# dvillacis/BPLDenoising

Hardware: AMD Instinct MI355X
Metric: PDHG iters/sec (batched 128x128 images) (higher is better)
Workload: dtype f64; 1 GPU; 10x128x128 f64 batch, scalar alpha, 5000 PDHG iterations per step (denoise); images_per_gpu=10, tile_iters=8, tiles_per_launch=490, hipgraph=True, parallelism=images of one batch sharded, dp1

## Files before the change

bpldenoising_amd/csrc/pdhg_kernels.hpp:

```cpp
#pragma once
#include <hip/hip_runtime.h>

#include "tiling.hpp"

namespace bpltv {

constexpr size_t pdhg_lds_bytes(int RI, int RJ, size_t word = sizeof(double)) {
    return word * ((size_t)RJ * (RI + 1) + (size_t)(RJ + 1) * RI + (size_t)RJ * RI + RI + 1);
}

constexpr int TAB_STRIDE = 8;

struct PdhgArgs {
    const double* xin;
    const double* y1in;
    const double* y2in;
    double* xout;
    double* y1out;
    double* y2out;
    const double* f;
    const double* alpha;
    const double* tab;
    double rho;
    int am, an;
    int it0, nit;
    int M, N, O;
    int nTi, nTj, halo;
    int first;
    int img0;
    int Odata;
    int astride;
    int istride;
    int ntiles;
    int grid3d;
    int seg;
    int xcd;
    unsigned* phase = nullptr;
#ifdef BPLTV_EXPERIMENTS
    int dbg;
#endif
};

#ifdef BPLTV_EXPERIMENTS
#define BPLTV_DBG(A) ((A).dbg)
__device__ long long pdhg_tlog[2][4096];
#define PDHG_TLOG(A)                                                                                                   \
    if (((A).dbg & 1024) && threadIdx.x == 0 && blockIdx.x == 0 && blockIdx.y == 0 && blockIdx.z == 0)                  \
        pdhg_tlog[(A).img0 != 0][min(4095, ((A).it0 + (A).halo - 1) / max((A).halo, 1))] = (long long)wall_clock64();
#else
#define BPLTV_DBG(A) 0
#define PDHG_TLOG(A)
#endif

#define PDHG_PHASE_STAMP(A)                                                                              \
    if ((A).phase != nullptr && threadIdx.x == 0 && blockIdx.x == 0 && blockIdx.y == 0 && blockIdx.z == 0) \
        *(A).phase = (unsigned)(A).it0 + 1u;
#define PDHG_DECODE_BLOCK(A, imgl, ta, tb)                                   \
    PDHG_PHASE_STAMP(A)                                                      \
    PDHG_TLOG(A)                                                             \
    int imgl, ta, tb;                                                        \
    if ((A).grid3d) {                                                        \
        ta = (int)blockIdx.x; tb = (int)blockIdx.y; imgl = (int)blockIdx.z;  \
    } else {                                                                 \
        const int tilesPerImg_ = (A).nTi * (A).nTj;                          \
        int lin_ = (int)blockIdx.x;                                          \
        if ((A).xcd) {                                                       \
            const int q_ = (int)gridDim.x >> 3, r_ = (int)gridDim.x & 7;     \
            const int x_ = lin_ & 7, i_ = lin_ >> 3;                         \
            lin_ = x_ * q_ + (x_ < r_ ? x_ : r_) + i_;                       \
        }                                                                    \
        imgl = lin_ / tilesPerImg_;                                          \
        const int t_ = lin_ - imgl * tilesPerImg_;                           \
        ta = t_ % (A).nTi; tb = t_ / (A).nTi;                                \
    }
__device__ __forceinline__ size_t pdhg_data_image(const PdhgArgs& A, int img, int& fimg) {
    if (A.O == A.Odata) { fimg = img; return (size_t)img * A.istride; }
    fimg = img % A.Odata;
    return (size_t)(img / A.Odata) * A.astride;
}

__device__ __forceinline__ double alpha_at(const double* __restrict__ alpha, int am, int an, int M,
                                           int N, int i, int j) {
    if (am == 1 && an == 1) return alpha[0];
    if (am == M && an == N) return alpha[i + (size_t)M * j];
    return alpha[(int)(((long)i * am) / M) + (size_t)am * (int)(((long)j * an) / N)];
}

__device__ __forceinline__ double rsqrt_nr(double n2) {
    const unsigned long long u = 0x5FE6EB50C7B537A9ull - ((unsigned long long)__double_as_longlong(n2) >> 1);
    double r = __longlong_as_double((long long)u);
    const double h = 0.5 * n2;
#pragma unroll
    for (int k = 0; k < 4; ++k) {
        const double t = r * r;
        const double w = __builtin_fma(-h, t, 1.5);
        r = r * w;
    }
    return r;
}

__device__ __forceinline__ float rsqrt_nr(float n2) {
    const unsigned u = 0x5F375A86u - (__float_as_uint(n2) >> 1);
    float r = __uint_as_float(u);
    const float h = 0.5f * n2;
#pragma unroll
    for (int k = 0; k < 3; ++k) {
        const float t = r * r;
        const float w = __builtin_fmaf(-h, t, 1.5f);
        r = r * w;
    }
    return r;
}
__device__ __forceinline__ void rsqrt_nr_seed(double n2, double& r, double& h) {
    const unsigned long long u = 0x5FE6EB50C7B537A9ull - ((unsigned long long)__double_as_longlong(n2) >> 1);
    r = __longlong_as_double((long long)u);
    h = 0.5 * n2;
}
__device__ __forceinline__ void rsqrt_nr_seed(float n2, float& r, float& h) {
    r = __uint_as_float(0x5F375A86u - (__float_as_uint(n2) >> 1));
    h = 0.5f * n2;
}
__host__ __device__ constexpr int rsqrt_nr_steps(double) { return 4; }
__host__ __device__ constexpr int rsqrt_nr_steps(float) { return 3; }
__device__ __forceinline__ double pd_fma(double a, double b, double c) { return __builtin_fma(a, b, c); }
__device__ __forceinline__ float pd_fma(float a, float b, float c) { return __builtin_fmaf(a, b, c); }

template <typename T, int PI, int PJ, int TI, int TJ>
__global__ __launch_bounds__(TI* TJ) void pdhg_tile_kernel(PdhgArgs A) {
    constexpr int RI = PI * TI, RJ = PJ * TJ;
    constexpr int S1 = RI + 1;
    extern __shared__ __attribute__((aligned(16))) unsigned char pdhg_smem[];
    T* smem = reinterpret_cast<T*>(pdhg_smem);
    T* sy1 = smem;
    T* sy2 = smem + RJ * S1;
    T* sxb = smem + RJ * S1 + (RJ + 1) * RI;
    const T* __restrict__ Axin = reinterpret_cast<const T*>(A.xin);
    const T* __restrict__ Ay1in = reinterpret_cast<const T*>(A.y1in);
    const T* __restrict__ Ay2in = reinterpret_cast<const T*>(A.y2in);
    T* __restrict__ Axout = reinterpret_cast<T*>(A.xout);
    T* __restrict__ Ay1out = reinterpret_cast<T*>(A.y1out);
    T* __restrict__ Ay2out = reinterpret_cast<T*>(A.y2out);
    const T* __restrict__ Af = reinterpret_cast<const T*>(A.f);

    const int tid = threadIdx.x;
    const int ti = tid % TI, tj = tid / TI;
    PDHG_DECODE_BLOCK(A, imgl, ta, tb)
    const int img = A.img0 + imgl;
    int oi, ci0, ci1, oj, cj0, cj1;
    tile_span(ta, A.M, RI, A.halo, oi, ci0, ci1);
    tile_span(tb, A.N, RJ, A.halo, oj, cj0, cj1);
    const int M = A.M, N = A.N;
    int fimg;
    const size_t aoff = pdhg_data_image(A, img, fimg);
    const size_t base = (size_t)img * M * N;
    const size_t fbase = (size_t)fimg * M * N;
    const T* __restrict__ alpha = reinterpret_cast<const T*>(A.alpha) + aoff;
    const int amode = (A.am == 1 && A.an == 1) ? 0 : ((A.am == M && A.an == N) ? 2 : 1);
    const bool first = (A.first != 0) || (BPLTV_DBG(A) & 1);

    T x[PJ][PI], y1[PJ][PI], y2[PJ][PI], f[PJ][PI], al[PJ][PI];
    size_t gidx[PJ][PI], fidx[PJ][PI], aidx[PJ][PI];
#pragma unroll
    for (int pj = 0; pj < PJ; ++pj)
#pragma unroll
        for (int pi = 0; pi < PI; ++pi) {
            const int li = ti + TI * pi, lj = PJ * tj + pj;
            const int gi = min(oi + li, M - 1), gj = min(oj + lj, N - 1);
            gidx[pj][pi] = base + gi + (size_t)M * gj;
            fidx[pj][pi] = fbase + gi + (size_t)M * gj;
            size_t ai = 0;
            if (amode == 2) {
                ai = gi + (size_t)M * gj;
            } else if (amode == 1) {
                const unsigned pa = ((unsigned)gi * (unsigned)A.am) / (unsigned)M;
                const unsigned pb = ((unsigned)gj * (unsigned)A.an) / (unsigned)N;
                ai = pa + (size_t)A.am * pb;
            }
            aidx[pj][pi] = ai;
        }
    if (!first) {
#pragma unroll
        for (int pj = 0; pj < PJ; ++pj)
#pragma unroll
            for (int pi = 0; pi < PI; ++pi) {
                if (BPLTV_DBG(A) & 64) {
                    x[pj][pi] = __builtin_nontemporal_load(&Axin[gidx[pj][pi]]);
                    y1[pj][pi] = __builtin_nontemporal_load(&Ay1in[gidx[pj][pi]]);
                    y2[pj][pi] = __builtin_nontemporal_load(&Ay2in[gidx[pj][pi]]);
                } else {
                    x[pj][pi] = Axin[gidx[pj][pi]];
                    y1[pj][pi] = Ay1in[gidx[pj][pi]];
                    y2[pj][pi] = Ay2in[gidx[pj][pi]];
                }
            }
    }
#pragma unroll
    for (int pj = 0; pj < PJ; ++pj)
#pragma unroll
        for (int pi = 0; pi < PI; ++pi) {
            f[pj][pi] = Af[fidx[pj][pi]];
            al[pj][pi] = alpha[aidx[pj][pi]];
        }
#pragma unroll
    for (int pj = 0; pj < PJ; ++pj)
#pragma unroll
        for (int pi = 0; pi < PI; ++pi) {
            const int li = ti + TI * pi, lj = PJ * tj + pj;
            const bool in = (oi + li < M) && (oj + lj < N);
            if (first) {
                x[pj][pi] = f[pj][pi];
                y1[pj][pi] = T(0);
                y2[pj][pi] = T(0);
            }
            if (!in) {
                f[pj][pi] = T(0); x[pj][pi] = T(0); y1[pj][pi] = T(0); y2[pj][pi] = T(0); al[pj][pi] = T(0);
            }
            sy1[lj * S1 + li + 1] = y1[pj][pi];
            sy2[(lj + 1) * RI + li] = y2[pj][pi];
        }
    for (int e = threadIdx.x; e < RJ; e += TI * TJ) sy1[e * S1] = T(0);
    for (int e = threadIdx.x; e < RI; e += TI * TJ) sy2[e] = T(0);
    for (int e = threadIdx.x; e < RI + 1; e += TI * TJ) sxb[RI * RJ + e] = T(0);
    __syncthreads();

    const T rho = (T)A.rho;
    const int nit = (BPLTV_DBG(A) & 4) ? 0 : A.nit;
    int n1[PJ][PI], n2[PJ][PI];
#pragma unroll
    for (int pj = 0; pj < PJ; ++pj)
#pragma unroll
        for (int pi = 0; pi < PI; ++pi) {
            const int li = ti + TI * pi, lj = PJ * tj + pj;
            const int l = lj * RI + li;
            n1[pj][pi] = l + (((oi + li) < M - 1) ? 1 : 0);
            n2[pj][pi] = l + (((oj + lj) < N - 1) ? RI : 0);
        }
    int my_nit = nit;
    if (PI * PJ > 1 && N > RJ) {
        const int w0 = (tid & ~63) / TI, w1 = min((tid | 63) / TI, TJ - 1);
        const int r0 = PJ * w0, r1 = PJ * w1 + PJ - 1;
        if (oj > 0) my_nit = min(my_nit, r1);
        if (oj + RJ < N) my_nit = min(my_nit, RJ - r0);
    }
    const T* __restrict__ row = reinterpret_cast<const T*>(A.tab) + (size_t)TAB_STRIDE * A.it0;
    T tau = row[0], sigma = row[1], omega = row[2], inv1ptau = row[3], opw = row[4];
    for (int it = 0; it < nit; ++it) {
        const T* __restrict__ nrow = row + TAB_STRIDE * ((it + 1 < nit) ? it + 1 : it);
        const T ntau = nrow[0], nsigma = nrow[1], nomega = nrow[2], ninv1ptau = nrow[3], nopw = nrow[4];
        const bool act = it < my_nit;
        T xb[PJ][PI];
        T y1m[PJ][PI], y2m[PJ][PI];
        if (act) {
#pragma unroll
        for (int pj = 0; pj < PJ; ++pj)
#pragma unroll
            for (int pi = 0; pi < PI; ++pi) {
                const int li = ti + TI * pi, lj = PJ * tj + pj;
                y1m[pj][pi] = sy1[lj * S1 + li];
                y2m[pj][pi] = sy2[lj * RI + li];
            }
#pragma unroll
        for (int pj = 0; pj < PJ; ++pj)
#pragma unroll
            for (int pi = 0; pi < PI; ++pi) {
                const int li = ti + TI * pi, lj = PJ * tj + pj;
                const int l = lj * RI + li;
                const T div = (y1m[pj][pi] - y1[pj][pi]) + (y2m[pj][pi] - y2[pj][pi]);
                const T tt = div - f[pj][pi];
                const T xo = x[pj][pi];
                const T xn = pd_fma(-tau, tt, xo) * inv1ptau;
                const T b = pd_fma(-omega, xo, opw * xn);
                x[pj][pi] = xn;
                xb[pj][pi] = b;
                sxb[l] = b;
            }
        }
        __syncthreads();
        if (act) {
        T xp1[PJ][PI], xpM[PJ][PI];
#pragma unroll
        for (int pj = 0; pj < PJ; ++pj)
#pragma unroll
            for (int pi = 0; pi < PI; ++pi) {
                xp1[pj][pi] = sxb[n1[pj][pi]];
                xpM[pj][pi] = sxb[n2[pj][pi]];
            }
        T n2v[PJ][PI];
        bool any_out = false;
#pragma unroll
        for (int pj = 0; pj < PJ; ++pj)
#pragma unroll
            for (int pi = 0; pi < PI; ++pi) {
                const T b = xb[pj][pi];
                const T d1 = xp1[pj][pi] - b;
                const T d2 = xpM[pj][pi] - b;
                const T a = al[pj][pi];
                T y1n = pd_fma(sigma, d1, y1[pj][pi]);
                T y2n = pd_fma(sigma, d2, y2[pj][pi]);
                if (rho != T(0)) {
                    const T den = T(1) + sigma * rho / a;
                    y1n = y1n / den;
                    y2n = y2n / den;
                }
                y1[pj][pi] = y1n;
                y2[pj][pi] = y2n;
                n2v[pj][pi] = pd_fma(y2n, y2n, y1n * y1n);
                any_out |= n2v[pj][pi] > a * a;
            }
        if (any_out) {
#pragma unroll
            for (int pj = 0; pj < PJ; ++pj)
#pragma unroll
                for (int pi = 0; pi < PI; ++pi) {
                    const T a = al[pj][pi];
                    const T v = a * rsqrt_nr(n2v[pj][pi]);
                    const bool outp = n2v[pj][pi] > a * a;
                    y1[pj][pi] = outp ? y1[pj][pi] * v : y1[pj][pi];
                    y2[pj][pi] = outp ? y2[pj][pi] * v : y2[pj][pi];
                }
        }
#pragma unroll
        for (int pj = 0; pj < PJ; ++pj)
#pragma unroll
            for (int pi = 0; pi < PI; ++pi) {
                const int li = ti + TI * pi, lj = PJ * tj + pj;
                sy1[lj * S1 + li + 1] = y1[pj][pi];
                sy2[(lj + 1) * RI + li] = y2[pj][pi];
            }
        }
        tau = ntau; sigma = nsigma; omega = nomega; inv1ptau = ninv1ptau; opw = nopw;
        __syncthreads();
    }

#pragma unroll
    for (int pj = 0; pj < PJ; ++pj)
#pragma unroll
        for (int pi = 0; pi < PI; ++pi) {
            const int li = ti + TI * pi, lj = PJ * tj + pj;
            const int gi = oi + li, gj = oj + lj;
            if (gi >= ci0 && gi < ci1 && gj >= cj0 && gj < cj1 && !(BPLTV_DBG(A) & 2)) {
                const size_t idx = base + gi + (size_t)M * gj;
                if (BPLTV_DBG(A) & 16) {
                    __builtin_nontemporal_store(x[pj][pi], &Axout[idx]);
                    __builtin_nontemporal_store(y1[pj][pi], &Ay1out[idx]);
                    __builtin_nontemporal_store(y2[pj][pi], &Ay2out[idx]);
                } else if (!(BPLTV_DBG(A) & 32)) {
                    __hip_atomic_store(&Axout[idx], x[pj][pi], __ATOMIC_RELAXED, __HIP_MEMORY_SCOPE_AGENT);
                    __hip_atomic_store(&Ay1out[idx], y1[pj][pi], __ATOMIC_RELAXED, __HIP_MEMORY_SCOPE_AGENT);
                    __hip_atomic_store(&Ay2out[idx], y2[pj][pi], __ATOMIC_RELAXED, __HIP_MEMORY_SCOPE_AGENT);
                } else {
                    Axout[idx] = x[pj][pi];
                    Ay1out[idx] = y1[pj][pi];
                    Ay2out[idx] = y2[pj][pi];
                }
            }
        }
}

template <typename T>
__device__ __forceinline__ T pd_shfl(T v, int src) { return __shfl(v, src, 64); }
__device__ __forceinline__ int pd_dpp_prev(int v) { return __builtin_amdgcn_update_dpp(v, v, 0x138, 0xf, 0xf, false); }
__device__ __forceinline__ int pd_dpp_next(int v) { return __builtin_amdgcn_update_dpp(v, v, 0x130, 0xf, 0xf, false); }
__device__ __forceinline__ double pd_lane_prev(double v) {
    return __hiloint2double(pd_dpp_prev(__double2hiint(v)), pd_dpp_prev(__double2loint(v)));
}
__device__ __forceinline__ double pd_lane_next(double v) {
    return __hiloint2double(pd_dpp_next(__double2hiint(v)), pd_dpp_next(__double2loint(v)));
}
__device__ __forceinline__ float pd_lane_prev(float v) { return __int_as_float(pd_dpp_prev(__float_as_int(v))); }
__device__ __forceinline__ float pd_lane_next(float v) { return __int_as_float(pd_dpp_next(__float_as_int(v))); }

__device__ __forceinline__ double pd_lane_prev_or0(double v) {
    return __hiloint2double(__builtin_amdgcn_update_dpp(0, __double2hiint(v), 0x138, 0xf, 0xf, true),
                            __builtin_amdgcn_update_dpp(0, __double2loint(v), 0x138, 0xf, 0xf, true));
}
__device__ __forceinline__ double pd_lane_next_or_self(double v) {
    return __hiloint2double(__builtin_amdgcn_update_dpp(__double2hiint(v), __double2hiint(v), 0x130, 0xf, 0xf, false),
                            __builtin_amdgcn_update_dpp(__double2loint(v), __double2loint(v), 0x130, 0xf, 0xf, false));
}
__device__ __forceinline__ double pd_lane_prev_or(double v, double fill) {
    return __hiloint2double(__builtin_amdgcn_update_dpp(__double2hiint(fill), __double2hiint(v), 0x138, 0xf, 0xf, false),
                            __builtin_amdgcn_update_dpp(__double2loint(fill), __double2loint(v), 0x138, 0xf, 0xf, false));
}
__device__ __forceinline__ double pd_lane_next_or(double v, double fill) {
    return __hiloint2double(__builtin_amdgcn_update_dpp(__double2hiint(fill), __double2hiint(v), 0x130, 0xf, 0xf, false),
                            __builtin_amdgcn_update_dpp(__double2loint(fill), __double2loint(v), 0x130, 0xf, 0xf, false));
}
__device__ __forceinline__ float pd_lane_prev_or(float v, float fill) {
    return __int_as_float(__builtin_amdgcn_update_dpp(__float_as_int(fill), __float_as_int(v), 0x138, 0xf, 0xf, false));
}
__device__ __forceinline__ float pd_lane_next_or(float v, float fill) {
    return __int_as_float(__builtin_amdgcn_update_dpp(__float_as_int(fill), __float_as_int(v), 0x130, 0xf, 0xf, false));
}
__device__ __forceinline__ float pd_lane_prev_or0(float v) {
    return __int_as_float(__builtin_amdgcn_update_dpp(0, __float_as_int(v), 0x138, 0xf, 0xf, true));
}
__device__ __forceinline__ float pd_lane_next_or_self(float v) {
    return __int_as_float(__builtin_amdgcn_update_dpp(__float_as_int(v), __float_as_int(v), 0x130, 0xf, 0xf, false));
}

constexpr size_t pdhg_rows_lds(int PJ, int TJ, bool CL, size_t word = sizeof(double)) {
    return word * 64 * (2 * (size_t)(TJ + 1) + (CL ? 2 * (size_t)PJ * TJ : 0));
}

template <typename T, int PJ, int TJ, bool CL>
__global__ __launch_bounds__(64 * TJ) void pdhg_rows_kernel(PdhgArgs A) {
    constexpr int RI = 64, RJ = PJ * TJ;
    extern __shared__ __attribute__((aligned(16))) unsigned char pdhg_smem[];
    T* sy2 = reinterpret_cast<T*>(pdhg_smem);
    T* sxb = sy2 + (TJ + 1) * 64;
    T* sfc = sxb + (TJ + 1) * 64;
    const T* __restrict__ Axin = reinterpret_cast<const T*>(A.xin);
    const T* __restrict__ Ay1in = reinterpret_cast<const T*>(A.y1in);
    const T* __restrict__ Ay2in = reinterpret_cast<const T*>(A.y2in);
    T* __restrict__ Axout = reinterpret_cast<T*>(A.xout);
    T* __restrict__ Ay1out = reinterpret_cast<T*>(A.y1out);
    T* __restrict__ Ay2out = reinterpret_cast<T*>(A.y2out);
    const T* __restrict__ Af = reinterpret_cast<const T*>(A.f);
    const int tid = threadIdx.x, ti = tid & 63;
    const int tj = __builtin_amdgcn_readfirstlane(tid >> 6);
    PDHG_DECODE_BLOCK(A, imgl, ta, tb)
#ifdef BPLTV_EXPERIMENTS
    if ((BPLTV_DBG(A) >> 8) > 0) {
        const unsigned lin = blockIdx.x + gridDim.x * (blockIdx.y + gridDim.y * blockIdx.z);
        if (lin < 512u) {
            const unsigned hsh = (lin * 2654435761u) >> 16;
            const int units = (int)(hsh % (unsigned)(BPLTV_DBG(A) >> 8));
            for (int k = 0; k < units; ++k) __builtin_amdgcn_s_sleep(16);
        }
    }
#endif
    const int img = A.img0 + imgl;
    int oi, ci0, ci1, oj, cj0, cj1;
    tile_span(ta, A.M, RI, A.halo, oi, ci0, ci1);
    tile_span(tb, A.N, RJ, A.halo, oj, cj0, cj1);
    const int M = A.M, N = A.N;
    int fimg;
    const size_t aoff = pdhg_data_image(A, img, fimg);
    const size_t base = (size_t)img * M * N;
    const size_t fbase = (size_t)fimg * M * N;
    const T* __restrict__ alpha = reinterpret_cast<const T*>(A.alpha) + aoff;
    const int amode = (A.am == 1 && A.an == 1) ? 0 : ((A.am == M && A.an == N) ? 2 : 1);
    const bool first = (A.first != 0) || (BPLTV_DBG(A) & 1);
    const int lj0 = PJ * tj;
    const int gi = min(oi + ti, M - 1);
    const bool in_i = oi + ti < M;

    T x[PJ], y1[PJ], y2[PJ], f[PJ], al[PJ];
#pragma unroll
    for (int pj = 0; pj < PJ; ++pj) {
        const int gj = min(oj + lj0 + pj, N - 1);
        const size_t gidx = gi + (size_t)M * gj;
        size_t ai = 0;
        if (amode == 2) ai = gidx;
        else if (amode == 1) ai = ((unsigned)gi * (unsigned)A.am) / (unsigned)M + (size_t)A.am * (((unsigned)gj * (unsigned)A.an) / (unsigned)N);
        if (!first) {
            x[pj] = Axin[base + gidx];
            y1[pj] = Ay1in[base + gidx];
            y2[pj] = Ay2in[base + gidx];
        }
        f[pj] = Af[fbase + gidx];
        al[pj] = alpha[ai];
    }
#pragma unroll
    for (int pj = 0; pj < PJ; ++pj) {
        if (first) { x[pj] = f[pj]; y1[pj] = T(0); y2[pj] = T(0); }
        if (!(in_i && oj + lj0 + pj < N)) { f[pj] = T(0); x[pj] = T(0); y1[pj] = T(0); y2[pj] = T(0); al[pj] = T(0); }
        if (CL) {
            sfc[(lj0 + pj) * 64 + ti] = f[pj];
            sfc[(RJ + lj0 + pj) * 64 + ti] = al[pj];
        }
    }
    sy2[(tj + 1) * 64 + ti] = y2[PJ - 1];
    if (tj == 0) { sy2[ti] = T(0); sxb[TJ * 64 + ti] = T(0); }
    __syncthreads();

    const T rho = (T)A.rho;
    const int nit = A.nit;
    const bool hasD_last = oj + lj0 + PJ - 1 < N - 1;
    int lim[PJ];
#pragma unroll
    for (int pj = 0; pj < PJ; ++pj) {
        const int lj = lj0 + pj;
        int l = nit;
// ... 1070 lines not shown
```

bpldenoising_amd/csrc/sumregs_kernels.hpp:

```cpp
#pragma once
#include <hip/hip_runtime.h>
#include "pdhg_kernels.hpp"

namespace bpltv {

constexpr size_t sr_lds_bytes(int RI, int RJ) { return sizeof(double) * (7 * (size_t)RI * RJ + 1); }

struct SrArgs {
    const double* in[7];
    double* out[7];
    const double* f;
    const double* alpha;
    const double* tab;
    double rho;
    int am, an;
    int it0, nit;
    int M, N, O;
    int nTi, nTj, halo;
    int first;
    int img0;
    int Odata;
    int astride;
};

__device__ __forceinline__ size_t sr_alpha_index(int am, int an, int M, int N, int i, int j) {
    if (am == 1 && an == 1) return 0;
    if (am == M && an == N) return i + (size_t)M * j;
    return (size_t)(((unsigned)i * (unsigned)am) / (unsigned)M) + (size_t)am * (((unsigned)j * (unsigned)an) / (unsigned)N);
}

template <int TI, int TJ, bool SWEEP = false>
__global__ __launch_bounds__(TI* TJ) void sr_tile_kernel(SrArgs A) {
    constexpr int RI = TI, RJ = TJ, RN = RI * RJ;
    extern __shared__ __attribute__((aligned(16))) double smem[];
    double* sy = smem;
    double* sxb = smem + 6 * RN;
    const int tid = threadIdx.x;
    const int li = tid % TI, lj = tid / TI;
    const int ta = (int)blockIdx.x, tb = (int)blockIdx.y;
    const int img = A.img0 + (int)blockIdx.z;
    int oi, ci0, ci1, oj, cj0, cj1;
    tile_span(ta, A.M, RI, A.halo, oi, ci0, ci1);
    tile_span(tb, A.N, RJ, A.halo, oj, cj0, cj1);
    const int M = A.M, N = A.N;
    int fimg = img, apar = 0;
    if (SWEEP) { fimg = (int)((unsigned)img % (unsigned)A.Odata); apar = (int)((unsigned)img / (unsigned)A.Odata); }
    const size_t base = (size_t)img * M * N;
    const double* __restrict__ fsrc = A.f + (size_t)fimg * M * N;
    const double* __restrict__ alpha = A.alpha + (size_t)apar * A.astride;
    const int gi = oi + li, gj = oj + lj;
    const bool in = gi < M && gj < N;
    const int ci = min(gi, M - 1), cj = min(gj, N - 1);
    const size_t q = ci + (size_t)M * cj, g = base + q;
    const size_t ai = sr_alpha_index(A.am, A.an, M, N, ci, cj), sl = (size_t)A.am * A.an;
    double x, f, y[6], al[3];
    f = fsrc[q];
    al[0] = alpha[ai]; al[1] = alpha[sl + ai]; al[2] = alpha[2 * sl + ai];
    if (!A.first) {
        x = A.in[0][g];
#pragma unroll
        for (int c = 0; c < 6; ++c) y[c] = A.in[1 + c][g];
    } else {
        x = f;
#pragma unroll
        for (int c = 0; c < 6; ++c) y[c] = 0.0;
    }
    if (!in) {
        x = 0.0; f = 0.0;
#pragma unroll
        for (int c = 0; c < 6; ++c) y[c] = 0.0;
        al[0] = al[1] = al[2] = 0.0;
    }
    const int l = lj * RI + li;
    const bool hasL = gi > 0, hasR = gi < M - 1, hasU = gj > 0, hasD = gj < N - 1;
    const int nim = l - ((hasL && li > 0) ? 1 : 0), nip = l + ((hasR && li < RI - 1) ? 1 : 0);
    const int njm = l - ((hasU && lj > 0) ? RI : 0), njp = l + ((hasD && lj < RJ - 1) ? RI : 0);
    const int zf1m = hasL ? nim : (7 - 0) * RN, zf2m = hasU ? njm : (7 - 1) * RN;
    const int zb1p = hasR ? nip : (7 - 2) * RN, zb2p = hasD ? njp : (7 - 3) * RN;
    if (tid == 0) smem[7 * RN] = 0.0;
#pragma unroll
    for (int c = 0; c < 6; ++c) sy[c * RN + l] = y[c];
    __syncthreads();

    const double rho = A.rho;
    const double* __restrict__ row = A.tab + (size_t)TAB_STRIDE * A.it0;
    double tau = row[0], sigma = row[1], omega = row[2], inv1ptau = row[3], opw = row[4];
    for (int it = 0; it < A.nit; ++it) {
        const double* __restrict__ nrow = row + TAB_STRIDE * ((it + 1 < A.nit) ? it + 1 : it);
        const double ntau = nrow[0], nsigma = nrow[1], nomega = nrow[2], ninv1ptau = nrow[3], nopw = nrow[4];
        const double f1m = sy[0 * RN + zf1m], f2m = sy[1 * RN + zf2m];
        const double b1p = sy[2 * RN + zb1p], b2p = sy[3 * RN + zb2p];
        const double c1m = sy[4 * RN + nim], c1p = sy[4 * RN + nip];
        const double c2m = sy[5 * RN + njm], c2p = sy[5 * RN + njp];
        const double tf = (f1m - y[0]) + (f2m - y[1]);
        const double tbk = (y[2] - b1p) + (y[3] - b2p);
        const double ca = hasL ? c1m : -y[4], cb = hasR ? c1p : -y[4];
        const double cc = hasU ? c2m : -y[5], cd = hasD ? c2p : -y[5];
        const double tc = 0.5 * (ca - cb) + 0.5 * (cc - cd);
        const double div = (tf + tbk) + tc;
        const double tt = div - f;
        const double xo = x;
        const double xn = __builtin_fma(-tau, tt, xo) * inv1ptau;
        const double bc = __builtin_fma(-omega, xo, opw * xn);
        x = xn;
        sxb[l] = bc;
        __syncthreads();
        const double bp = sxb[nip], bm = sxb[nim], cp = sxb[njp], cm = sxb[njm];
        double d1[3], d2[3];
        d1[0] = bp - bc; d2[0] = cp - bc;
        d1[1] = bc - bm; d2[1] = bc - cm;
        d1[2] = 0.5 * (bp - bm); d2[2] = 0.5 * (cp - cm);
        double n2v[3];
        bool any_out = false;
#pragma unroll
        for (int k = 0; k < 3; ++k) {
            const double a = al[k];
            double y1n = __builtin_fma(sigma, d1[k], y[2 * k]);
            double y2n = __builtin_fma(sigma, d2[k], y[2 * k + 1]);
            if (rho != 0.0) {
                const double den = 1.0 + sigma * rho / a;
                y1n = y1n / den;
                y2n = y2n / den;
            }
            y[2 * k] = y1n;
            y[2 * k + 1] = y2n;
            n2v[k] = __builtin_fma(y2n, y2n, y1n * y1n);
            any_out |= n2v[k] > a * a;
        }
        (void)any_out;
#pragma unroll
        for (int k = 0; k < 3; ++k) {
            const double a = al[k];
            if (n2v[k] > a * a) {
                const double v = a * rsqrt_nr(n2v[k]);
                y[2 * k] = y[2 * k] * v;
                y[2 * k + 1] = y[2 * k + 1] * v;
            }
        }
#pragma unroll
        for (int c = 0; c < 6; ++c) sy[c * RN + l] = y[c];
        tau = ntau; sigma = nsigma; omega = nomega; inv1ptau = ninv1ptau; opw = nopw;
        __syncthreads();
    }
    if (gi >= ci0 && gi < ci1 && gj >= cj0 && gj < cj1) {
        const size_t idx = base + gi + (size_t)M * gj;
        __hip_atomic_store(&A.out[0][idx], x, __ATOMIC_RELAXED, __HIP_MEMORY_SCOPE_AGENT);
#pragma unroll
        for (int c = 0; c < 6; ++c) __hip_atomic_store(&A.out[1 + c][idx], y[c], __ATOMIC_RELAXED, __HIP_MEMORY_SCOPE_AGENT);
    }
}

template <int PJ, int TI, int TJ, bool SWEEP = false>
__global__ __launch_bounds__(TI* TJ) void sr_strip_kernel(SrArgs A) {
    constexpr int RI = TI, RJ = PJ * TJ, RN = RI * RJ;
    extern __shared__ __attribute__((aligned(16))) double smem[];
    double* sy = smem;
    double* sxb = smem + 6 * RN;
    const int tid = threadIdx.x;
    const int li = tid % TI, tj = tid / TI, lj0 = PJ * tj;
    const int ta = (int)blockIdx.x, tb = (int)blockIdx.y;
    const int img = A.img0 + (int)blockIdx.z;
    int oi, ci0, ci1, oj, cj0, cj1;
    tile_span(ta, A.M, RI, A.halo, oi, ci0, ci1);
    tile_span(tb, A.N, RJ, A.halo, oj, cj0, cj1);
    const int M = A.M, N = A.N;
    int fimg = img, apar = 0;
    if (SWEEP) { fimg = (int)((unsigned)img % (unsigned)A.Odata); apar = (int)((unsigned)img / (unsigned)A.Odata); }
    const size_t base = (size_t)img * M * N;
    const double* __restrict__ fsrc = A.f + (size_t)fimg * M * N;
    const double* __restrict__ alpha = A.alpha + (size_t)apar * A.astride;
    const int gi = oi + li, ci = min(gi, M - 1);
    const size_t sl = (size_t)A.am * A.an;
    double x[PJ], f[PJ], y[PJ][6], al[PJ][3], bc[PJ];
    size_t g[PJ];
    bool hasU[PJ], hasD[PJ];
#pragma unroll
    for (int pj = 0; pj < PJ; ++pj) {
        const int gj = oj + lj0 + pj, cj = min(gj, N - 1);
        const size_t q = ci + (size_t)M * cj;
        g[pj] = base + q;
        const size_t ai = sr_alpha_index(A.am, A.an, M, N, ci, cj);
        f[pj] = fsrc[q];
        al[pj][0] = alpha[ai]; al[pj][1] = alpha[sl + ai]; al[pj][2] = alpha[2 * sl + ai];
        if (!A.first) {
            x[pj] = A.in[0][g[pj]];
#pragma unroll
            for (int c = 0; c < 6; ++c) y[pj][c] = A.in[1 + c][g[pj]];
        }
    }
#pragma unroll
    for (int pj = 0; pj < PJ; ++pj) {
        const int gj = oj + lj0 + pj;
        if (A.first) {
            x[pj] = f[pj];
#pragma unroll
            for (int c = 0; c < 6; ++c) y[pj][c] = 0.0;
        }
        if (!(gi < M && gj < N)) {
            x[pj] = 0.0; f[pj] = 0.0;
#pragma unroll
            for (int c = 0; c < 6; ++c) y[pj][c] = 0.0;
            al[pj][0] = al[pj][1] = al[pj][2] = 0.0;
        }
        hasU[pj] = gj > 0;
        hasD[pj] = gj < N - 1;
    }
    const bool hasL = gi > 0, hasR = gi < M - 1;
    const int l0 = lj0 * RI + li, lE = l0 + (PJ - 1) * RI;
    const int dm = (hasL && li > 0) ? -1 : 0, dp = (hasR && li < RI - 1) ? 1 : 0;
    const bool upIn = hasU[0] && lj0 > 0, dnIn = hasD[PJ - 1] && lj0 + PJ < RJ;
    const int upC = upIn ? l0 - RI : l0, dnC = dnIn ? lE + RI : lE;
    const int upF = hasU[0] ? (upIn ? l0 - RI : lE) : (7 - 1) * RN;
    const int dnB = hasD[PJ - 1] ? (dnIn ? lE + RI : l0) : (7 - 3) * RN;
    const int zdm = hasL ? dm : (7 - 0) * RN - l0, zdp = hasR ? dp : (7 - 2) * RN - l0;
    if (tid == 0) smem[7 * RN] = 0.0;
    auto store_duals = [&]() {
#pragma unroll
        for (int pj = 0; pj < PJ; ++pj) {
            const int l = l0 + pj * RI;
            sy[0 * RN + l] = y[pj][0];
            sy[2 * RN + l] = y[pj][2];
            sy[4 * RN + l] = y[pj][4];
            if (pj == PJ - 1) sy[1 * RN + l] = y[pj][1];
            if (pj == 0) sy[3 * RN + l] = y[pj][3];
            if (pj == 0 || pj == PJ - 1) sy[5 * RN + l] = y[pj][5];
        }
    };
    store_duals();
    __syncthreads();

    const double rho = A.rho;
    const double* __restrict__ row = A.tab + (size_t)TAB_STRIDE * A.it0;
    double tau = row[0], sigma = row[1], omega = row[2], inv1ptau = row[3], opw = row[4];
    for (int it = 0; it < A.nit; ++it) {
        const double* __restrict__ nrow = row + TAB_STRIDE * ((it + 1 < A.nit) ? it + 1 : it);
        const double ntau = nrow[0], nsigma = nrow[1], nomega = nrow[2], ninv1ptau = nrow[3], nopw = nrow[4];
#pragma unroll
        for (int pj = 0; pj < PJ; ++pj) {
            const int l = l0 + pj * RI;
            const double f1m = sy[0 * RN + (hasL ? l : l0) + zdm], b1p = sy[2 * RN + (hasR ? l : l0) + zdp];
            const double c1m = sy[4 * RN + l + dm], c1p = sy[4 * RN + l + dp];
            const double f2m = (pj > 0) ? y[pj > 0 ? pj - 1 : 0][1] : sy[1 * RN + upF];
            const double c2m = (pj > 0) ? y[pj > 0 ? pj - 1 : 0][5] : sy[5 * RN + upC];
            const bool hU = hasU[pj], hD = hasD[pj];
            const double b2p = (pj < PJ - 1) ? (hD ? y[pj < PJ - 1 ? pj + 1 : pj][3] : 0.0) : sy[3 * RN + dnB];
            const double c2p = (pj < PJ - 1) ? y[pj < PJ - 1 ? pj + 1 : pj][5] : sy[5 * RN + dnC];
            const double tf = (f1m - y[pj][0]) + (f2m - y[pj][1]);
            const double tbk = (y[pj][2] - b1p) + (y[pj][3] - b2p);
            const double ca = hasL ? c1m : -y[pj][4], cb = hasR ? c1p : -y[pj][4];
            const double cc = hU ? c2m : -y[pj][5], cd = hD ? c2p : -y[pj][5];
            const double tc = 0.5 * (ca - cb) + 0.5 * (cc - cd);
            const double div = (tf + tbk) + tc;
            const double tt = div - f[pj];
            const double xo = x[pj];
            const double xn = __builtin_fma(-tau, tt, xo) * inv1ptau;
            bc[pj] = __builtin_fma(-omega, xo, opw * xn);
            x[pj] = xn;
            sxb[l] = bc[pj];
        }
        __syncthreads();
#pragma unroll
        for (int pj = 0; pj < PJ; ++pj) {
            const int l = l0 + pj * RI;
            const double bcc = bc[pj];
            const double bp = sxb[l + dp], bm = sxb[l + dm];
            const double cp = (pj < PJ - 1) ? (hasD[pj] ? bc[pj < PJ - 1 ? pj + 1 : pj] : bcc) : sxb[dnC];
            const double cm = (pj > 0) ? bc[pj > 0 ? pj - 1 : 0] : sxb[upC];
            double d1[3], d2[3];
            d1[0] = bp - bcc; d2[0] = cp - bcc;
            d1[1] = bcc - bm; d2[1] = bcc - cm;
            d1[2] = 0.5 * (bp - bm); d2[2] = 0.5 * (cp - cm);
            double n2v[3];
            bool any_out = false;
#pragma unroll
            for (int k = 0; k < 3; ++k) {
                const double a = al[pj][k];
                double y1n = __builtin_fma(sigma, d1[k], y[pj][2 * k]);
                double y2n = __builtin_fma(sigma, d2[k], y[pj][2 * k + 1]);
                if (rho != 0.0) {
                    const double den = 1.0 + sigma * rho / a;
                    y1n = y1n / den;
                    y2n = y2n / den;
                }
                y[pj][2 * k] = y1n;
                y[pj][2 * k + 1] = y2n;
                n2v[k] = __builtin_fma(y2n, y2n, y1n * y1n);
                any_out |= n2v[k] > a * a;
            }
            (void)any_out;
#pragma unroll
            for (int k = 0; k < 3; ++k) {
                const double a = al[pj][k];
                if (n2v[k] > a * a) {
                    const double v = a * rsqrt_nr(n2v[k]);
                    y[pj][2 * k] = y[pj][2 * k] * v;
                    y[pj][2 * k + 1] = y[pj][2 * k + 1] * v;
                }
            }
        }
        store_duals();
        tau = ntau; sigma = nsigma; omega = nomega; inv1ptau = ninv1ptau; opw = nopw;
        __syncthreads();
    }
#pragma unroll
    for (int pj = 0; pj < PJ; ++pj) {
        const int gj = oj + lj0 + pj;
        if (gi >= ci0 && gi < ci1 && gj >= cj0 && gj < cj1) {
            __hip_atomic_store(&A.out[0][g[pj]], x[pj], __ATOMIC_RELAXED, __HIP_MEMORY_SCOPE_AGENT);
#pragma unroll
            for (int c = 0; c < 6; ++c) __hip_atomic_store(&A.out[1 + c][g[pj]], y[pj][c], __ATOMIC_RELAXED, __HIP_MEMORY_SCOPE_AGENT);
        }
    }
}

struct SrCoef {
    double *t1, *t2, *c, *kap, *h1, *h2, *rhs;
    size_t tot;
};

constexpr double SR_ACT_TOL = 1e-12;

__device__ __forceinline__ void sr_grad_at(int k, const double* __restrict__ v, int M, int N, int i, int j, double& d1, double& d2) {
    const size_t q = i + (size_t)M * j;
    const double uc = v[q];
    const double up = v[(i < M - 1) ? q + 1 : q], um = v[(i > 0) ? q - 1 : q];
    const double vp = v[(j < N - 1) ? q + M : q], vm = v[(j > 0) ? q - M : q];
    if (k == 0) { d1 = up - uc; d2 = vp - uc; }
    else if (k == 1) { d1 = uc - um; d2 = uc - vm; }
    else { d1 = 0.5 * (up - um); d2 = 0.5 * (vp - vm); }
}

__device__ __forceinline__ double sr_gradT_at(int k, const double* __restrict__ y1, const double* __restrict__ y2, int M, int N, int i,
                                              int j) {
    const size_t q = i + (size_t)M * j;
    if (k == 0) {
        const double a = (i > 0) ? y1[q - 1] : 0.0, b = (i < M - 1) ? y1[q] : 0.0;
        const double c = (j > 0) ? y2[q - M] : 0.0, d = (j < N - 1) ? y2[q] : 0.0;
        return (a - b) + (c - d);
    }
    if (k == 1) {
        const double a = (i > 0) ? y1[q] : 0.0, b = (i < M - 1) ? y1[q + 1] : 0.0;
        const double c = (j > 0) ? y2[q] : 0.0, d = (j < N - 1) ? y2[q + M] : 0.0;
        return (a - b) + (c - d);
    }
    const double a = (i > 0) ? y1[q - 1] : -y1[q], b = (i < M - 1) ? y1[q + 1] : -y1[q];
    const double c = (j > 0) ? y2[q - M] : -y2[q], d = (j < N - 1) ? y2[q + M] : -y2[q];
    return 0.5 * (a - b) + 0.5 * (c - d);
}

struct SrState { const double* pl[7]; };
__global__ __launch_bounds__(256) void sr_gap_partial_kernel(SrState S, const double* __restrict__ f, const double* __restrict__ alpha,
                                                             int am, int an, int M, int N, double* __restrict__ partial) {
    __shared__ double sh[4];
    const int npx = M * N;
    const size_t base = (size_t)blockIdx.y * npx;
    const double* u = S.pl[0] + base;
    const size_t asl = (size_t)am * an;
    double s0 = 0.0, s1 = 0.0, s2 = 0.0, s3 = 0.0;
    for (int q = blockIdx.x * 256 + threadIdx.x; q < npx; q += gridDim.x * 256) {
        const int i = q % M, j = q / M;
        const double uk = u[q], fk = f[base + q];
        const size_t ai = sr_alpha_index(am, an, M, N, i, j);
        double w = 0.0, tv = 0.0;
#pragma unroll
        for (int k = 0; k < 3; ++k) {
            double d1, d2;
            sr_grad_at(k, u, M, N, i, j, d1, d2);
            tv += alpha[(size_t)k * asl + ai] * sqrt(d1 * d1 + d2 * d2);
        }
        w = (sr_gradT_at(0, S.pl[1] + base, S.pl[2] + base, M, N, i, j) + sr_gradT_at(1, S.pl[3] + base, S.pl[4] + base, M, N, i, j)) +
            sr_gradT_at(2, S.pl[5] + base, S.pl[6] + base, M, N, i, j);
        const double r = uk - fk;
        s0 += r * r;
        s1 += tv;
        s2 += fk * fk;
        s3 += (fk - w) * (fk - w);
    }
    s0 = block_sum<256>(s0, sh);
    s1 = block_sum<256>(s1, sh);
    s2 = block_sum<256>(s2, sh);
    s3 = block_sum<256>(s3, sh);
    if (threadIdx.x == 0) {
        double* p = partial + ((size_t)blockIdx.y * gridDim.x + blockIdx.x) * 4;
        p[0] = s0; p[1] = s1; p[2] = s2; p[3] = s3;
    }
}

template <bool COT>
__device__ __forceinline__ void sr_adj_setup_body(const double* __restrict__ u, const double* __restrict__ src,
                                                  const double* __restrict__ alpha, int am, int an, int M, int N, int O,
                                                  int patch, int reg, double kappa_act, SrCoef C) {
    const size_t npx = (size_t)M * N;
    const size_t e = (size_t)blockIdx.x * 256 + threadIdx.x;
    if (e >= npx * O) return;
    const int img = (int)(e / npx), k0 = (int)(e - (size_t)img * npx);
    const int i = k0 % M, j = k0 / M;
    const double* ui = u + (size_t)img * npx;
    const size_t ai = sr_alpha_index(am, an, M, N, i, j), astride = (size_t)am * an;
    const double gamma = patch ? 1e8 : 1e3;
#pragma unroll
    for (int k = 0; k < 3; ++k) {
        double g1, g2;
        sr_grad_at(k, ui, M, N, i, j, g1, g2);
        const double ng = sqrt(g1 * g1 + g2 * g2);
        const double a = alpha[k * astride + ai];
        double t1 = 0.0, t2 = 0.0, c = 0.0, kap = 0.0, h1 = 0.0, h2 = 0.0;
        if (!reg) {
            if (ng < SR_ACT_TOL) {
                kap = kappa_act;
            } else {
                t1 = -g2 / ng; t2 = g1 / ng;
                c = a / ng;
                h1 = g1 / ng; h2 = g2 / ng;
            }
        } else {
            if (ng > 1.0 / gamma) {
                t1 = -g2 / ng; t2 = g1 / ng;
                c = patch ? 1.0 / ng : a / ng;
                h1 = g1 / ng; h2 = g2 / ng;
            } else {
                kap = patch ? gamma : a * gamma;
                h1 = gamma * g1; h2 = gamma * g2;
            }
        }
        const size_t o = (size_t)k * C.tot + e;
        C.t1[o] = t1; C.t2[o] = t2; C.c[o] = c; C.kap[o] = kap; C.h1[o] = h1; C.h2[o] = h2;
    }
    if (COT) C.rhs[e] = reg ? -src[e] : src[e];
    else C.rhs[e] = reg ? src[e] - u[e] : u[e] - src[e];
}

__global__ __launch_bounds__(256) void sr_adj_setup_kernel(const double* __restrict__ u, const double* __restrict__ ubar,
                                                           const double* __restrict__ alpha, int am, int an, int M, int N, int O,
                                                           int patch, int reg, double kappa_act, SrCoef C) {
    sr_adj_setup_body<false>(u, ubar, alpha, am, an, M, N, O, patch, reg, kappa_act, C);
}

__global__ __launch_bounds__(256) void sr_adj_setup_cot_kernel(const double* __restrict__ u, const double* __restrict__ gu,
                                                               const double* __restrict__ alpha, int am, int an, int M, int N,
                                                               int O, int patch, int reg, double kappa_act, SrCoef C) {
    sr_adj_setup_body<true>(u, gu, alpha, am, an, M, N, O, patch, reg, kappa_act, C);
}

__global__ __launch_bounds__(256) void sr_adj_gradf_kernel(const double* __restrict__ p, size_t n, int reg,
                                                           double* __restrict__ grad_f) {
    const size_t q = (size_t)blockIdx.x * 256 + threadIdx.x;
    if (q >= n) return;
    grad_f[q] = reg ? -p[q] : p[q];
}

struct SrStencil { int pl[2], mi[2]; double s[2]; };
__device__ __forceinline__ SrStencil sr_stencil(int k, int M, int N, int i, int j) {
    const int q = i + M * j;
    SrStencil S;
    if (k == 0) {
        S.pl[0] = (i < M - 1) ? q + 1 : q; S.mi[0] = q; S.s[0] = (i < M - 1) ? 1.0 : 0.0;
        S.pl[1] = (j < N - 1) ? q + M : q; S.mi[1] = q; S.s[1] = (j < N - 1) ? 1.0 : 0.0;
    } else if (k == 1) {
        S.pl[0] = q; S.mi[0] = (i > 0) ? q - 1 : q; S.s[0] = (i > 0) ? 1.0 : 0.0;
        S.pl[1] = q; S.mi[1] = (j > 0) ? q - M : q; S.s[1] = (j > 0) ? 1.0 : 0.0;
    } else {
        S.pl[0] = (i < M - 1) ? q + 1 : q; S.mi[0] = (i > 0) ? q - 1 : q; S.s[0] = (S.pl[0] != S.mi[0]) ? 0.5 : 0.0;
        S.pl[1] = (j < N - 1) ? q + M : q; S.mi[1] = (j > 0) ? q - M : q; S.s[1] = (S.pl[1] != S.mi[1]) ? 0.5 : 0.0;
// ... 128 lines not shown
```

Measured before the change: 908,500 PDHG iterations/s of ONE 10x128x128 f64 batch.

## Stage step-size table rows in LDS and pin kernel args in SGPRs

Per-iteration step parameters (tau, sigma, omega, etc.) are loaded cooperatively into an LDS staging table 16 rows at a time, instead of every thread reading the next row from global memory each iteration. The per-iteration trailing barrier moves to the top of the loop so it also covers the staging write. Empty asm constraints keep kernel-argument pointers and scalars in SGPRs, and outputs use global address-space pointers. Launch bounds gain a minimum waves-per-SIMD hint, which may trade register headroom for occupancy.

```diff
diff --git a/bpldenoising_amd/csrc/pdhg_kernels.hpp b/bpldenoising_amd/csrc/pdhg_kernels.hpp
--- a/bpldenoising_amd/csrc/pdhg_kernels.hpp
+++ b/bpldenoising_amd/csrc/pdhg_kernels.hpp
@@ -5,11 +5,26 @@
 
 namespace bpltv {
 
+constexpr int TAB_STRIDE = 8;
+constexpr int STAB_ROWS = 16, STAB_COLS = 5;
+enum { STAB_TAU = 0, STAB_OMEGA = 1, STAB_INV1PTAU = 2, STAB_OPW = 3, STAB_SIGMA = 4 };
+__device__ __forceinline__ bool step_rows_lane(int it, int nit) {
+    const int t = threadIdx.x;
+    return t < 8 * STAB_ROWS && (t & 7) < STAB_COLS && it + (t >> 3) < nit;
+}
+template <typename T>
+__device__ __forceinline__ T step_rows_load(const T* __restrict__ tab, int it, int nit) {
+    return step_rows_lane(it, nit) ? tab[(size_t)TAB_STRIDE * it + threadIdx.x] : T(0);
+}
+template <typename T>
+__device__ __forceinline__ void step_rows_store(T* stab, T v, int it, int nit) {
+    const int r = threadIdx.x >> 3, c = threadIdx.x & 7;
+    if (step_rows_lane(it, nit)) stab[STAB_COLS * r + (c == 1 ? STAB_SIGMA : c - (c > 1))] = v;
+}
+
 constexpr size_t pdhg_lds_bytes(int RI, int RJ, size_t word = sizeof(double)) {
-    return word * ((size_t)RJ * (RI + 1) + (size_t)(RJ + 1) * RI + (size_t)RJ * RI + RI + 1);
-}
-
-constexpr int TAB_STRIDE = 8;
+    return word * ((size_t)RJ * (RI + 1) + (size_t)(RJ + 1) * RI + (size_t)RJ * RI + RI + 1 + STAB_ROWS * STAB_COLS);
+}
 
 struct PdhgArgs {
     const double* xin;
@@ -55,6 +70,9 @@
 #define PDHG_PHASE_STAMP(A)                                                                              \
     if ((A).phase != nullptr && threadIdx.x == 0 && blockIdx.x == 0 && blockIdx.y == 0 && blockIdx.z == 0) \
         *(A).phase = (unsigned)(A).it0 + 1u;
+#define PDHG_PIN_KERNARGS(A)                                                                                         \
+    asm volatile("" ::"s"((A).xin), "s"((A).y1in), "s"((A).y2in), "s"((A).f), "s"((A).alpha), "s"((A).tab), "s"((A).xout), \
+                 "s"((A).y1out), "s"((A).y2out), "s"((A).rho));
 #define PDHG_DECODE_BLOCK(A, imgl, ta, tb)                                   \
     PDHG_PHASE_STAMP(A)                                                      \
     PDHG_TLOG(A)                                                             \
@@ -125,8 +143,12 @@
 __device__ __forceinline__ double pd_fma(double a, double b, double c) { return __builtin_fma(a, b, c); }
 __device__ __forceinline__ float pd_fma(float a, float b, float c) { return __builtin_fmaf(a, b, c); }
 
+constexpr int pdhg_tile_waves(int px, int threads) {
+    const int per_simd = ((threads + 63) / 64 + 3) / 4;
+    return px <= 3 && threads >= 768 ? 2 * per_simd : 1;
+}
 template <typename T, int PI, int PJ, int TI, int TJ>
-__global__ __launch_bounds__(TI* TJ) void pdhg_tile_kernel(PdhgArgs A) {
+__global__ __launch_bounds__(TI* TJ, pdhg_tile_waves(PI* PJ, TI* TJ)) void pdhg_tile_kernel(PdhgArgs A) {
     constexpr int RI = PI * TI, RJ = PJ * TJ;
     constexpr int S1 = RI + 1;
     extern __shared__ __attribute__((aligned(16))) unsigned char pdhg_smem[];
@@ -134,6 +156,8 @@
     T* sy1 = smem;
     T* sy2 = smem + RJ * S1;
     T* sxb = smem + RJ * S1 + (RJ + 1) * RI;
+    T* stab = sxb + RJ * RI + RI + 1;
+    static_assert(8 * STAB_ROWS <= TI * TJ, "one staging lane per table word");
     const T* __restrict__ Axin = reinterpret_cast<const T*>(A.xin);
     const T* __restrict__ Ay1in = reinterpret_cast<const T*>(A.y1in);
     const T* __restrict__ Ay2in = reinterpret_cast<const T*>(A.y2in);
@@ -144,6 +168,7 @@
 
     const int tid = threadIdx.x;
     const int ti = tid % TI, tj = tid / TI;
+    PDHG_PIN_KERNARGS(A)
     PDHG_DECODE_BLOCK(A, imgl, ta, tb)
     const int img = A.img0 + imgl;
     int oi, ci0, ci1, oj, cj0, cj1;
@@ -178,6 +203,9 @@
             }
             aidx[pj][pi] = ai;
         }
+    const int nit = (BPLTV_DBG(A) & 4) ? 0 : A.nit;
+    const T* __restrict__ tab = reinterpret_cast<const T*>(A.tab) + (size_t)TAB_STRIDE * A.it0;
+    const T tab0 = step_rows_load(tab, 0, nit);
     if (!first) {
 #pragma unroll
         for (int pj = 0; pj < PJ; ++pj)
@@ -218,13 +246,12 @@
             sy1[lj * S1 + li + 1] = y1[pj][pi];
             sy2[(lj + 1) * RI + li] = y2[pj][pi];
         }
+    step_rows_store(stab, tab0, 0, nit);
     for (int e = threadIdx.x; e < RJ; e += TI * TJ) sy1[e * S1] = T(0);
     for (int e = threadIdx.x; e < RI; e += TI * TJ) sy2[e] = T(0);
     for (int e = threadIdx.x; e < RI + 1; e += TI * TJ) sxb[RI * RJ + e] = T(0);
-    __syncthreads();
 
     const T rho = (T)A.rho;
-    const int nit = (BPLTV_DBG(A) & 4) ? 0 : A.nit;
     int n1[PJ][PI], n2[PJ][PI];
 #pragma unroll
     for (int pj = 0; pj < PJ; ++pj)
@@ -242,11 +269,11 @@
         if (oj > 0) my_nit = min(my_nit, r1);
         if (oj + RJ < N) my_nit = min(my_nit, RJ - r0);
     }
-    const T* __restrict__ row = reinterpret_cast<const T*>(A.tab) + (size_t)TAB_STRIDE * A.it0;
-    T tau = row[0], sigma = row[1], omega = row[2], inv1ptau = row[3], opw = row[4];
-    for (int it = 0; it < nit; ++it) {
-        const T* __restrict__ nrow = row + TAB_STRIDE * ((it + 1 < nit) ? it + 1 : it);
-        const T ntau = nrow[0], nsigma = nrow[1], nomega = nrow[2], ninv1ptau = nrow[3], nopw = nrow[4];
+    for (int it = 0; it < nit;) {
+    const int itb = min(nit, it + STAB_ROWS);
+    for (const T* row = stab; it < itb; ++it, row += STAB_COLS) {
+        __syncthreads();
+        const T tau = row[STAB_TAU], omega = row[STAB_OMEGA], inv1ptau = row[STAB_INV1PTAU], opw = row[STAB_OPW];
         const bool act = it < my_nit;
         T xb[PJ][PI];
         T y1m[PJ][PI], y2m[PJ][PI];
@@ -277,6 +304,7 @@
         }
         __syncthreads();
         if (act) {
+        const T sigma = row[STAB_SIGMA];
         T xp1[PJ][PI], xpM[PJ][PI];
 #pragma unroll
         for (int pj = 0; pj < PJ; ++pj)
@@ -328,8 +356,8 @@
                 sy2[(lj + 1) * RI + li] = y2[pj][pi];
             }
         }
-        tau = ntau; sigma = nsigma; omega = nomega; inv1ptau = ninv1ptau; opw = nopw;
-        __syncthreads();
+    }
+    if (itb < nit) step_rows_store(stab, step_rows_load(tab, itb, nit), itb, nit);
     }
 
 #pragma unroll
diff --git a/bpldenoising_amd/csrc/sumregs_kernels.hpp b/bpldenoising_amd/csrc/sumregs_kernels.hpp
--- a/bpldenoising_amd/csrc/sumregs_kernels.hpp
+++ b/bpldenoising_amd/csrc/sumregs_kernels.hpp
@@ -4,7 +4,7 @@
 
 namespace bpltv {
 
-constexpr size_t sr_lds_bytes(int RI, int RJ) { return sizeof(double) * (7 * (size_t)RI * RJ + 1); }
+constexpr size_t sr_lds_bytes(int RI, int RJ) { return sizeof(double) * (7 * (size_t)RI * RJ + 1 + STAB_ROWS * STAB_COLS); }
 
 struct SrArgs {
     const double* in[7];
@@ -23,6 +23,19 @@
     int astride;
 };
 
+#define SR_PIN_KERNARGS(A)                                                                                              \
+    asm volatile("" ::"s"((A).in[0]), "s"((A).in[1]), "s"((A).in[2]), "s"((A).in[3]), "s"((A).in[4]), "s"((A).in[5]),     \
+                 "s"((A).in[6]), "s"((A).f), "s"((A).alpha), "s"((A).tab), "s"((A).rho));                                 \
+    asm volatile("" ::"s"((A).am), "s"((A).an), "s"((A).it0), "s"((A).nit), "s"((A).M), "s"((A).N), "s"((A).halo),         \
+                 "s"((A).first), "s"((A).img0));
+typedef __attribute__((address_space(1))) double* sr_gptr;
+#define SR_PIN_OUT(A, out)                                                                                              \
+    double* out##_[7] = {(A).out[0], (A).out[1], (A).out[2], (A).out[3], (A).out[4], (A).out[5], (A).out[6]};             \
+    asm volatile("" : "+s"(out##_[0]), "+s"(out##_[1]), "+s"(out##_[2]), "+s"(out##_[3]), "+s"(out##_[4]),               \
+                 "+s"(out##_[5]), "+s"(out##_[6]));                                                                      \
+    const sr_gptr out[7] = {(sr_gptr)out##_[0], (sr_gptr)out##_[1], (sr_gptr)out##_[2], (sr_gptr)out##_[3],               \
+                            (sr_gptr)out##_[4], (sr_gptr)out##_[5], (sr_gptr)out##_[6]};
+
 __device__ __forceinline__ size_t sr_alpha_index(int am, int an, int M, int N, int i, int j) {
     if (am == 1 && an == 1) return 0;
     if (am == M && an == N) return i + (size_t)M * j;
@@ -30,13 +43,16 @@
 }
 
 template <int TI, int TJ, bool SWEEP = false>
-__global__ __launch_bounds__(TI* TJ) void sr_tile_kernel(SrArgs A) {
+__global__ __launch_bounds__(TI* TJ, 2 * (TI * TJ / 256)) void sr_tile_kernel(SrArgs A) {
     constexpr int RI = TI, RJ = TJ, RN = RI * RJ;
     extern __shared__ __attribute__((aligned(16))) double smem[];
     double* sy = smem;
     double* sxb = smem + 6 * RN;
+    double* stab = smem + 7 * RN + 1;
+    static_assert(8 * STAB_ROWS <= TI * TJ, "one staging lane per table word");
     const int tid = threadIdx.x;
     const int li = tid % TI, lj = tid / TI;
+    SR_PIN_KERNARGS(A)
     const int ta = (int)blockIdx.x, tb = (int)blockIdx.y;
     const int img = A.img0 + (int)blockIdx.z;
     int oi, ci0, ci1, oj, cj0, cj1;
@@ -54,6 +70,9 @@
     const size_t q = ci + (size_t)M * cj, g = base + q;
     const size_t ai = sr_alpha_index(A.am, A.an, M, N, ci, cj), sl = (size_t)A.am * A.an;
     double x, f, y[6], al[3];
+    const int nit = A.nit;
+    const double* __restrict__ tab = A.tab + (size_t)TAB_STRIDE * A.it0;
+    const double tab0 = step_rows_load(tab, 0, nit);
     f = fsrc[q];
     al[0] = alpha[ai]; al[1] = alpha[sl + ai]; al[2] = alpha[2 * sl + ai];
     if (!A.first) {
@@ -65,29 +84,30 @@
 #pragma unroll
         for (int c = 0; c < 6; ++c) y[c] = 0.0;
     }
+    SR_PIN_OUT(A, out)
     if (!in) {
         x = 0.0; f = 0.0;
 #pragma unroll
         for (int c = 0; c < 6; ++c) y[c] = 0.0;
         al[0] = al[1] = al[2] = 0.0;
     }
-    const int l = lj * RI + li;
+    const int l = tid;
     const bool hasL = gi > 0, hasR = gi < M - 1, hasU = gj > 0, hasD = gj < N - 1;
     const int nim = l - ((hasL && li > 0) ? 1 : 0), nip = l + ((hasR && li < RI - 1) ? 1 : 0);
     const int njm = l - ((hasU && lj > 0) ? RI : 0), njp = l + ((hasD && lj < RJ - 1) ? RI : 0);
     const int zf1m = hasL ? nim : (7 - 0) * RN, zf2m = hasU ? njm : (7 - 1) * RN;
     const int zb1p = hasR ? nip : (7 - 2) * RN, zb2p = hasD ? njp : (7 - 3) * RN;
     if (tid == 0) smem[7 * RN] = 0.0;
+    step_rows_store(stab, tab0, 0, nit);
 #pragma unroll
     for (int c = 0; c < 6; ++c) sy[c * RN + l] = y[c];
-    __syncthreads();
 
     const double rho = A.rho;
-    const double* __restrict__ row = A.tab + (size_t)TAB_STRIDE * A.it0;
-    double tau = row[0], sigma = row[1], omega = row[2], inv1ptau = row[3], opw = row[4];
-    for (int it = 0; it < A.nit; ++it) {
-        const double* __restrict__ nrow = row + TAB_STRIDE * ((it + 1 < A.nit) ? it + 1 : it);
-        const double ntau = nrow[0], nsigma = nrow[1], nomega = nrow[2], ninv1ptau = nrow[3], nopw = nrow[4];
+    for (int it = 0; it < nit;) {
+    const int itb = min(nit, it + STAB_ROWS);
+    for (const double* row = stab; it < itb; ++it, row += STAB_COLS) {
+        __syncthreads();
+        const double tau = row[STAB_TAU], omega = row[STAB_OMEGA], inv1ptau = row[STAB_INV1PTAU], opw = row[STAB_OPW];
         const double f1m = sy[0 * RN + zf1m], f2m = sy[1 * RN + zf2m];
         const double b1p = sy[2 * RN + zb1p], b2p = sy[3 * RN + zb2p];
         const double c1m = sy[4 * RN + nim], c1p = sy[4 * RN + nip];
@@ -105,6 +125,7 @@
         x = xn;
         sxb[l] = bc;
         __syncthreads();
+        const double sigma = row[STAB_SIGMA];
         const double bp = sxb[nip], bm = sxb[nim], cp = sxb[njp], cm = sxb[njm];
         double d1[3], d2[3];
         d1[0] = bp - bc; d2[0] = cp - bc;
@@ -139,14 +160,17 @@
         }
 #pragma unroll
         for (int c = 0; c < 6; ++c) sy[c * RN + l] = y[c];
-        tau = ntau; sigma = nsigma; omega = nomega; inv1ptau = ninv1ptau; opw = nopw;
-        __syncthreads();
-    }
-    if (gi >= ci0 && gi < ci1 && gj >= cj0 && gj < cj1) {
-        const size_t idx = base + gi + (size_t)M * gj;
-        __hip_atomic_store(&A.out[0][idx], x, __ATOMIC_RELAXED, __HIP_MEMORY_SCOPE_AGENT);
-#pragma unroll
-        for (int c = 0; c < 6; ++c) __hip_atomic_store(&A.out[1 + c][idx], y[c], __ATOMIC_RELAXED, __HIP_MEMORY_SCOPE_AGENT);
+    }
+    if (itb < nit) step_rows_store(stab, step_rows_load(tab, itb, nit), itb, nit);
+    }
+    int tid2 = threadIdx.x;
+    asm volatile("" : "+v"(tid2));
+    const int gi2 = oi + tid2 % TI, gj2 = oj + tid2 / TI;
+    if (gi2 >= ci0 && gi2 < ci1 && gj2 >= cj0 && gj2 < cj1) {
+        const size_t idx = base + gi2 + (size_t)M * gj2;
+        __hip_atomic_store(&out[0][idx], x, __ATOMIC_RELAXED, __HIP_MEMORY_SCOPE_AGENT);
+#pragma unroll
+        for (int c = 0; c < 6; ++c) __hip_atomic_store(&out[1 + c][idx], y[c], __ATOMIC_RELAXED, __HIP_MEMORY_SCOPE_AGENT);
     }
 }
 
@@ -156,8 +180,11 @@
     extern __shared__ __attribute__((aligned(16))) double smem[];
     double* sy = smem;
     double* sxb = smem + 6 * RN;
+    double* stab = smem + 7 * RN + 1;
+    static_assert(8 * STAB_ROWS <= TI * TJ, "one staging lane per table word");
     const int tid = threadIdx.x;
     const int li = tid % TI, tj = tid / TI, lj0 = PJ * tj;
+    SR_PIN_KERNARGS(A)
     const int ta = (int)blockIdx.x, tb = (int)blockIdx.y;
     const int img = A.img0 + (int)blockIdx.z;
     int oi, ci0, ci1, oj, cj0, cj1;
@@ -174,6 +201,9 @@
     double x[PJ], f[PJ], y[PJ][6], al[PJ][3], bc[PJ];
     size_t g[PJ];
     bool hasU[PJ], hasD[PJ];
+    const int nit = A.nit;
+    const double* __restrict__ tab = A.tab + (size_t)TAB_STRIDE * A.it0;
+    const double tab0 = step_rows_load(tab, 0, nit);
 #pragma unroll
     for (int pj = 0; pj < PJ; ++pj) {
         const int gj = oj + lj0 + pj, cj = min(gj, N - 1);
@@ -188,6 +218,7 @@
             for (int c = 0; c < 6; ++c) y[pj][c] = A.in[1 + c][g[pj]];
         }
     }
+    SR_PIN_OUT(A, out)
 #pragma unroll
     for (int pj = 0; pj < PJ; ++pj) {
         const int gj = oj + lj0 + pj;
@@ -227,14 +258,14 @@
         }
     };
     store_duals();
-    __syncthreads();
+    step_rows_store(stab, tab0, 0, nit);
 
     const double rho = A.rho;
-    const double* __restrict__ row = A.tab + (size_t)TAB_STRIDE * A.it0;
-    double tau = row[0], sigma = row[1], omega = row[2], inv1ptau = row[3], opw = row[4];
-    for (int it = 0; it < A.nit; ++it) {
-        const double* __restrict__ nrow = row + TAB_STRIDE * ((it + 1 < A.nit) ? it + 1 : it);
-        const double ntau = nrow[0], nsigma = nrow[1], nomega = nrow[2], ninv1ptau = nrow[3], nopw = nrow[4];
+    for (int it = 0; it < nit;) {
+    const int itb = min(nit, it + STAB_ROWS);
+    for (const double* row = stab; it < itb; ++it, row += STAB_COLS) {
+        __syncthreads();
+        const double tau = row[STAB_TAU], omega = row[STAB_OMEGA], inv1ptau = row[STAB_INV1PTAU], opw = row[STAB_OPW];
 #pragma unroll
         for (int pj = 0; pj < PJ; ++pj) {
             const int l = l0 + pj * RI;
@@ -259,6 +290,7 @@
             sxb[l] = bc[pj];
         }
         __syncthreads();
+        const double sigma = row[STAB_SIGMA];
 #pragma unroll
         for (int pj = 0; pj < PJ; ++pj) {
             const int l = l0 + pj * RI;
@@ -299,16 +331,16 @@
             }
         }
         store_duals();
-        tau = ntau; sigma = nsigma; omega = nomega; inv1ptau = ninv1ptau; opw = nopw;
-        __syncthreads();
+    }
+    if (itb < nit) step_rows_store(stab, step_rows_load(tab, itb, nit), itb, nit);
     }
 #pragma unroll
     for (int pj = 0; pj < PJ; ++pj) {
         const int gj = oj + lj0 + pj;
         if (gi >= ci0 && gi < ci1 && gj >= cj0 && gj < cj1) {
-            __hip_atomic_store(&A.out[0][g[pj]], x[pj], __ATOMIC_RELAXED, __HIP_MEMORY_SCOPE_AGENT);
-#pragma unroll
-            for (int c = 0; c < 6; ++c) __hip_atomic_store(&A.out[1 + c][g[pj]], y[pj][c], __ATOMIC_RELAXED, __HIP_MEMORY_SCOPE_AGENT);
+            __hip_atomic_store(&out[0][g[pj]], x[pj], __ATOMIC_RELAXED, __HIP_MEMORY_SCOPE_AGENT);
+#pragma unroll
+            for (int c = 0; c < 6; ++c) __hip_atomic_store(&out[1 + c][g[pj]], y[pj][c], __ATOMIC_RELAXED, __HIP_MEMORY_SCOPE_AGENT);
         }
     }
 }
```

After: 898,600 PDHG iterations/s of ONE 10x128x128 f64 batch. -1.1%, worse.
